# afalchetti/monorfs

Hardware: AMD Instinct MI355X
Metric: PHD updates/sec (particles x components x measurements) (higher is better)
Workload: dtype f64; 1 GPU; RB-PHD-SLAM SlamUpdate, BASELINE config B: 2048 particles/GPU x 512 components x 64 measurements, PRM3D pixel-range model, prior weights 'survey', state resident in HBM; particles_per_gpu=2048, components=512, measurements=64, max_quantity=600, parallelism=particles sharded x1

## Files before the change

### monorfs_amd/csrc/phd_alpha.h

```cpp
#pragma once
#include "phd_device.h"


__device__ __forceinline__ int pk_get(unsigned int perm, int i) { return (int) ((perm >> (4 * i)) & 15u); }

__device__ __forceinline__ unsigned int pk_set(unsigned int perm, int i, int v)
{
	return (perm & ~(15u << (4 * i))) | ((unsigned int) v << (4 * i));
}

__device__ __forceinline__ unsigned int pk_reverse(unsigned int perm, int from, int to)
{
	for (int i = from, j = to - 1; i < j; i++, j--) {
		int vi = pk_get(perm, i), vj = pk_get(perm, j);
		perm = pk_set(pk_set(perm, i, vj), j, vi);
	}
	return perm;
}

__device__ __forceinline__ bool pk_last(unsigned int perm, int n)
{
	for (int i = 1; i < n; i++) {
		if (pk_get(perm, i - 1) < pk_get(perm, i)) return false;
	}
// ... 360 lines not shown
	};
	auto store_node = [&](int slot, const int (&mx)[NT], unsigned int fr, int parent, int er, int ec) {
#pragma unroll
		for (int t = 0; t < NT; t++) {
			const int i = lane + 64 * t;
			if (i < n) nd.asg[(size_t) slot * nd.stride + i] = (unsigned char) mx[t];
			const unsigned long long w = ballot64((fr >> t) & 1u);
			if (lane == 0) nd.forced[slot * NT + t] = w;
		}
		int ne = 0;
		if (parent >= 0) {
			ne = nd.nelim[parent];
			for (int e = lane; e < ne; e += 64) nd.elist[slot * MURTY_ELCAP + e] = nd.elist[parent * MURTY_ELCAP + e];
		}
		if (lane == 0) {
			if (er >= 0 && ne < MURTY_ELCAP) nd.elist[slot * MURTY_ELCAP + ne] = (unsigned short) ((er << 8) | ec);
			nd.nelim[slot] = ne + ((er >= 0 && ne < MURTY_ELCAP) ? 1 : 0);
		}
		__threadfence_block();
	};

	{
		int slot = alloc();
		int mx[NT];
		bool solved = wave_hungarian<NT>(profit, n, lane, mx);
		if (!solved) {
#pragma unroll
			for (int t = 0; t < NT; t++) mx[t] = 0;
		}
		store_node(slot, mx, 0u, -1, -1, 0);
		double value = solved ? wave_assignment_value<NT>(profit, n, mx) : -INFINITY;
		frontier_add(value, solved ? slot : (slot | 0x10000));
	}

	while (fsize > 0) {
		const double value = ws.fkey[fsize - 1];
		const int    code  = ws.fnode[fsize - 1];
		fsize--;
		if (m >= MURTY_OUT || (ws.logcomp[m] - ws.logcomp[0] < -10)) break;
		if (lane == 0) ws.logcomp[m] = value;
		const int slot = code & 0xffff;
		hook(m, (code & 0x10000) != 0, [&](int row) { return (int) nd.asg[(size_t) slot * nd.stride + row]; });
		m++;
		lds_fence();
		if (code & 0x10000) continue;
		int pa[NT];
		unsigned int fr = 0, fc = 0;
		unsigned long long rem[NT];
		int R = 0;
#pragma unroll
		for (int t = 0; t < NT; t++) {
			const int i = lane + 64 * t;
			pa[t] = (i < n) ? nd.asg[(size_t) slot * nd.stride + i] : 0;
			const unsigned long long fw = nd.forced[slot * NT + t];
			if ((fw >> lane) & 1ull) fr |= 1u << t;
			const int left = n - 64 * t;
			const unsigned long long rows = (left >= 64) ? ~0ull : ((left <= 0) ? 0ull : ((1ull << left) - 1ull));
			rem[t] = ~fw & rows;
			R += __popcll(rem[t]);
		}
#pragma unroll
		for (int t = 0; t < NT; t++) {
			unsigned long long fw = ballot64((fr >> t) & 1u);
			while (fw) {
				const int l = __ffsll((long long) fw) - 1;
				fw &= fw - 1;
				const int col = __shfl(pa[t], l, 64);
				if (lane == (col & 63)) fc |= 1u << (col >> 6);
			}
		}
		const int pne = nd.nelim[slot];
		for (int c = 0; c < R - 1; c++) {
			int er = -1;
#pragma unroll
			for (int t = 0; t < NT; t++) {
				if (er < 0 && rem[t]) {
					er = 64 * t + __ffsll((long long) rem[t]) - 1;
					rem[t] &= rem[t] - 1;
				}
			}
			const int ec = spread_get<NT>(pa, er);
			for (int i = 0; i < n; i++) {
				const int  pai = spread_get<NT>(pa, i);
				const bool fi  = __shfl((int) fr, i & 63, 64) & (1 << (i >> 6));
#pragma unroll
				for (int t = 0; t < NT; t++) {
					const int k = lane + 64 * t;
					if (k < n) {
						double v = profit[i * n + k];
						if (fi) v = (k == pai) ? 1.0 : -INFINITY;
						else if ((fc >> t) & 1u) v = -INFINITY;
						nd.reduced[i * n + k] = v;
					}
				}
			}
			__threadfence_block();
			for (int e = lane; e < pne; e += 64) {
				const int ed = nd.elist[slot * MURTY_ELCAP + e];
				nd.reduced[(ed >> 8) * n + (ed & 255)] = -INFINITY;
			}
			if (lane == 0) nd.reduced[er * n + ec] = -INFINITY;
			__threadfence_block();
			int mx[NT];
			const bool solved = wave_hungarian<NT>(nd.reduced, n, lane, mx);
			if (solved) {
				const int cs = alloc();
				store_node(cs, mx, fr, slot, er, ec);
				frontier_add(wave_assignment_value<NT>(profit, n, mx), cs);
			}
			if (lane == (er & 63)) fr |= 1u << (er >> 6);
			if (lane == (ec & 63)) fc |= 1u << (ec >> 6);
		}
		if (lane == 0) ws.freelist[nfree] = slot;
		nfree++;
		lds_fence();
	}
	return m;
}

template <int TAG, class Hook>
__device__ __forceinline__ int wave_murty_any(const MurtyLds& ws, const MurtyWs& nd, int n, int lane, Hook hook)
{
	if (n <= 64) return wave_murty<1, TAG>(ws, nd, n, lane, hook);
	if (n <= 128) return wave_murty<2, TAG>(ws, nd, n, lane, hook);
	return wave_murty<4, TAG>(ws, nd, n, lane, hook);
}

__device__ void jacobian_p(const DevParams& prm, const PoseD& pose, const double m[3], double* Jp)
{
	if (prm.linear2d) {
		for (int i = 0; i < 18; i++) Jp[i] = 0.0;
		Jp[0] = -1.0; Jp[7] = -1.0;
		return;
	}
	const double diff[3] = {m[0] - pose.t[0], m[1] - pose.t[1], m[2] - pose.t[2]};
	double l[3];
	to_local(pose, diff, l);
	const double f = prm.focal;
	const double mag = ((l[2] > 0) ? 1.0 : -1.0) * sqrt(l[0] * l[0] + l[1] * l[1] + l[2] * l[2]);
	const double jp[9] = {f / l[2], 0, -f * l[0] / (l[2] * l[2]),  0, f / l[2], -f * l[1] / (l[2] * l[2]),
	                      l[0] / mag, l[1] / mag, l[2] / mag};
	double rc[9], jlocal[18];
	conj_matrix(pose, rc);
	const double cross[9] = {0, -diff[2], diff[1],  diff[2], 0, -diff[0],  -diff[1], diff[0], 0};
#pragma unroll
	for (int i = 0; i < 3; i++) {
#pragma unroll
		for (int j = 0; j < 3; j++) {
			double acc = 0;
#pragma unroll
			for (int k = 0; k < 3; k++) acc += (-1.0 * rc[i * 3 + k]) * cross[k * 3 + j];
			jlocal[i * 6 + j]     = -1.0 * rc[i * 3 + j];
			jlocal[i * 6 + 3 + j] = acc;
		}
	}
#pragma unroll
	for (int i = 0; i < 3; i++) {
#pragma unroll
		for (int j = 0; j < 6; j++) {
			double acc = 0;
#pragma unroll
			for (int k = 0; k < 3; k++) acc += jp[i * 3 + k] * jlocal[k * 6 + j];
			Jp[i * 6 + j] = acc;
		}
	}
}

__device__ __forceinline__ double pair_gradient(const DevParams& prm, const double* nu, const double* Jp, int t)
{
	double acc = 0;
#pragma unroll
	for (int b = 0; b < 3; b++) {
		double u = 0;
#pragma unroll
		for (int e = 0; e < 3; e++) u += nu[e] * prm.Rinv[e * 3 + b];
		acc += u * Jp[b * 6 + t];
	}
	return acc;
}

template <class Hook>
__device__ int cluster_enumerate_wave(const double* mat, int n, int modelsize, double* logcomp, int lane, Hook hook)
{
	int measurestart = n;
	for (int i = 0; i < n; i++) {
		if (i >= modelsize) { measurestart = i; break; }
	}
	unsigned int perm = pk_reverse(0x43210u, measurestart, n);
	int m = 0;
	for (;;) {
		double v = 0;
		for (int i = 0; i < n; i++) v += mat[i * 5 + pk_get(perm, i)];
		if (m < MURTY_OUT) {
			if (lane == 0) logcomp[m] = v;
			hook(m, perm);
			m++;
		}
		if (pk_last(perm, n)) break;
		perm = pk_next(perm, n, measurestart);
	}
	lds_fence();
	return m;
}

__global__ __launch_bounds__(64) void k_test_pairing(MurtyNodes* nodes, char* bigws, const double* matrix, int n, int mode, int modelsize,
                                                     int maxcount, int* assignments, double* values, int* count)
{
	__shared__ double lds[MURTY_LDS_DOUBLES + 2];
	const int lane = threadIdx.x;
	const MurtyLds ws = murty_lds(lds);
	const MurtyWs nd = (n <= MURTY_NMAX) ? murty_ws_particle(nodes) : murty_ws_carve(bigws, n);
	for (int i = lane; i < MURTY_OUT; i += 64) ws.logcomp[i] = 1e300;
	const int stride = (mode == 1) ? 5 : n;
	double* mat = (mode == 1) ? nd.reduced : nd.profit;
	for (int e = lane; e < n * n; e += 64) mat[(e / n) * stride + (e % n)] = matrix[e];
	lds_fence();
	int m;
	if (mode == 1) {
		m = cluster_enumerate_wave(mat, n, modelsize, ws.logcomp, lane, [&](int k, unsigned int perm) {
			if (k < maxcount && lane < n) assignments[k * n + lane] = pk_get(perm, lane);
		});
	}
	else {
		m = wave_murty_any<0>(ws, nd, n, lane, [&](int k, bool unsolved, auto colof) {
			if (k >= maxcount) return;
			for (int r = lane; r < n; r += 64) assignments[k * n + r] = unsolved ? -1 : colof(r);
		});
	}
	for (int k = lane; k < m && k < maxcount; k += 64) values[k] = ws.logcomp[k];
	if (lane == 0) *count = m;
}

#define ALPHA_JL 256

struct AlphaLds {
	int zs, red, lm, pick, scr;
	int p1_keyw, p1_sortw, p1_dw, p1_sortsrc, p1_selidx, ns;
	int p2_tile, p2_part;
	int p3_zh, p3_pdj, p3_lmd, p3_res, p3_adj, p3_adjT, p3_mem, p3_int, p3_x;
	int bytes;
};

__host__ __device__ inline AlphaLds alpha_lds(int MP, int ncap)
{
	const int JL = ALPHA_JL, MW = MP / 64;
	AlphaLds l;
	l.zs   = 0;
	l.red  = l.zs + 3 * MP;
	l.lm   = l.red + 256;
	l.pick = l.lm + 3 * JL;
	l.scr  = l.pick + JL / 2;
	int ns = 2;
	while (ns < ncap) ns <<= 1;
	l.ns = ns;
	l.p1_keyw = l.scr;
	l.p1_sortw = l.p1_keyw + ncap;
	l.p1_dw = l.p1_sortw + ns;
	l.p1_sortsrc = l.p1_dw + JL;
	l.p1_selidx = l.p1_sortsrc + (ns + JL + 1) / 2;
	int ph1 = l.p1_selidx + ns / 2 - l.scr;
	l.p2_tile = l.scr;
	l.p2_part = l.scr;
	int ph2 = 0;
	l.p3_zh = l.scr;
	l.p3_pdj = l.p3_zh + 3 * JL;
	l.p3_lmd = l.p3_pdj + JL;
	l.p3_res = l.p3_lmd + JL;
	l.p3_adj = l.p3_res + JL;
	l.p3_adjT = l.p3_adj + JL * MW;
	l.p3_mem = l.p3_adjT + MP * (JL / 64);
	l.p3_int = l.p3_mem + 2 * JL;
	l.p3_x   = l.p3_int + (3 * JL + MP + 1) / 2;
	int xs = 25 * 4 > MURTY_LDS_DOUBLES ? 25 * 4 : MURTY_LDS_DOUBLES;
	int ph3 = l.p3_x + xs + 2 - l.scr;
	int mx = ph1 > ph2 ? ph1 : ph2;
	mx = mx > ph3 ? mx : ph3;
	l.bytes = (l.scr + mx) * 8;
	return l;
}

#define QGRAD_WAVE_DOUBLES (25 + 5 * 18 + 120 * 6 + 120 + 9)
#define QGRAD_LDS_DOUBLES (4 * QGRAD_WAVE_DOUBLES)
#define QGRAD_G2_CLUSTERS 64
#define QGRAD_G2_WEIGHTS 384
#define QGRAD_HDR 10
#ifndef DENS_JL
#define DENS_JL 128
#endif
struct AlphaSlab {
	static constexpr int lm = 0, dw = 3, zh = 4, lpd = 7, res = 8, adj = 9, ints = 17, lmd = 19, memL = 20, memZ = 21, cnt = 22, total = 23;
	static constexpr int partc = 0, partp = 13;
	static constexpr int i_pick = 0, i_dsrc = 1, i_labl = 2, i_roots = 3;
	static constexpr int g_hdr = 0, g_jpall = g_hdr + QGRAD_HDR * ALPHA_JL, g_elist = g_jpall + 18 * ALPHA_JL;
};
static_assert(AlphaSlab::lm + 3 <= AlphaSlab::dw && AlphaSlab::dw + 1 <= AlphaSlab::zh && AlphaSlab::zh + 3 <= AlphaSlab::lpd &&
              AlphaSlab::lpd + 1 <= AlphaSlab::res && AlphaSlab::res + 1 <= AlphaSlab::adj && AlphaSlab::adj + 4 <= AlphaSlab::ints &&
              AlphaSlab::ints + (AlphaSlab::i_roots + 2) / 2 <= AlphaSlab::lmd && AlphaSlab::lmd + 1 <= AlphaSlab::memL &&
              AlphaSlab::memL + 1 <= AlphaSlab::memZ && AlphaSlab::memZ + 1 <= AlphaSlab::cnt && AlphaSlab::cnt + 1 <= AlphaSlab::total &&
              AlphaSlab::partc + 4 <= AlphaSlab::partp && AlphaSlab::partp + 4 <= AlphaSlab::total,
              "AlphaSlab: the Jcap-scaled arrays that are live together overlap, or pass the total");
__host__ __device__ inline size_t alpha_jscratch_doubles(int Jcap) { return (size_t) AlphaSlab::total * Jcap; }
__device__ __forceinline__ unsigned int my_xcd() { return __builtin_amdgcn_s_getreg((3 << 11) | 20) & 15u; }

template <int MW>
__device__ __forceinline__ bool has_detection(const unsigned long long* adj, int j)
{
	bool has = false;
#pragma unroll
	for (int b = 0; b < MW; b++) has |= adj[(size_t) j * MW + b] != 0;
	return has;
}

template <int ZB, bool QUASI, bool GRAD = false, int TAG = 0, bool DEPTH = false>
__device__ __forceinline__ void alpha_assoc_body(const DevParams& prm, const StepBufs& a, int ncap, double* smem, double* gws = nullptr,
                                                 int* helper_go = nullptr)
{
	constexpr int MP = ZB * 64;
	constexpr int MW = ZB;
	constexpr int JL = ALPHA_JL;
	const AlphaLds lay = alpha_lds(MP, ncap);
	double* zs   = smem + lay.zs;
	double* red  = smem + lay.red;
	double* etab = red;
	__shared__ int s_J, s_changed, s_nroots, s_big;
	__shared__ double s_ccount, s_total;
	__shared__ int s_ebump, s_g2lds;
	__shared__ double s_g2[GRAD ? QGRAD_G2_CLUSTERS * QGRAD_HDR + QGRAD_G2_WEIGHTS : 2];
	if (GRAD && threadIdx.x == 0) s_g2lds = 0;

	const int p = a.p0 + blockIdx.x, tid = threadIdx.x, lane = tid & 63, wv = tid >> 6;
	const int M = a.M, cap = a.cap;
	const MixView vout = bank_view(a, SEL_OUT);
	const Bank bin = bank_of(a, SEL_IN);
	const int no = QUASI ? 0 : vout.count[p];
	const size_t sbo = (size_t) p * cap;
	const PoseD pose = load_pose(QUASI ? a.qposes + (size_t) p * 7 : bin.poses + (size_t) p * 7);

	for (int k = tid; k < MP * 3; k += 256) zs[k] = (k < M * 3) ? a.z[k] : 0.0;
	unsigned int helper_word = 0;
	if (!QUASI && helper_go && tid == 0) helper_word = __hip_atomic_load(a.dsync + 3 * (size_t) p, __ATOMIC_RELAXED, __HIP_MEMORY_SCOPE_AGENT);

	PHD_STAMP_DECL;
	PHD_STAMP(0);
	double* keyw    = smem + lay.p1_keyw;
	double* sortw   = smem + lay.p1_sortw;
	int*    sortsrc = (int*) (smem + lay.p1_sortsrc);
	auto block_sum = [&](double v) {
		red[tid] = v;
		__syncthreads();
		for (int s = 128; s > 0; s >>= 1) {
			if (tid < s) red[tid] += red[tid + s];
			__syncthreads();
		}
		double r = red[0];
		__syncthreads();
		return r;
	};
	double wpart = 0;
	for (int c = tid; c < no; c += 256) {
		double wc = a.outw[sbo + c];
		keyw[c] = wc;
		wpart += wc;
	}
	{
		double e = block_sum(wpart);
		if (fabs(e - rint(e)) <= 1e-9 * fmax(1.0, fabs(e))) {
			if (tid == 0) {
				double q = 0;
				for (int c = 0; c < no; c++) q += keyw[c];
				s_ccount = q;
			}
			__syncthreads();
			e = s_ccount;
		}
		if (tid == 0) {
			s_ccount = e;
			int J = (int) e;
			if (J < 0) J = 0;
			if (J > a.Jcap) {
				atomicOr(a.flags, PHD_FLAG_J_OVERFLOW);
				J = a.Jcap;
			}
			s_J = QUASI ? min(a.qJ, a.Jcap) : J;
		}
	}
	PHD_STAMP(1);
	__syncthreads();
	const int J = s_J;
	if (J >= 1 && J <= no) {
		constexpr int HB = 500;
		int* const hist   = (int*) red;
		int* const selidx = (int*) (smem + lay.p1_selidx);
		int* const tl     = sortsrc;
		int& s_T = hist[HB];
		int& s_above = hist[HB + 1];
		int& s_nt = hist[HB + 2];
		int& s_ntaken = hist[HB + 3];
		const unsigned int hbase = (unsigned int) (((unsigned long long) __double_as_longlong(prm.minw) << 1) >> 49);
		auto bin_of = [&](double w) {
			const unsigned int k = (unsigned int) (((unsigned long long) __double_as_longlong(w) << 1) >> 49);
			return (int) min(max((int) k - (int) hbase, 0), HB - 1);
		};
		for (int t = tid; t < HB + 4; t += 256) hist[t] = 0;
		__syncthreads();
		for (int c = tid; c < no; c += 256) atomicAdd(&hist[bin_of(keyw[c])], 1);
		__syncthreads();
		if (wv == 0) {
			int cq[8], mine = 0;
#pragma unroll
			for (int q = 0; q < 8; q++) { const int b = 511 - (8 * lane + q); cq[q] = (b < HB) ? hist[b] : 0; mine += cq[q]; }
			int incl = mine;
#pragma unroll
			for (int o = 1; o < 64; o <<= 1) {
				const int y = __shfl_up(incl, o, 64);
				if (lane >= o) incl += y;
			}
			int run = incl - mine;
#pragma unroll
			for (int q = 0; q < 8; q++) {
				if (run < J && J <= run + cq[q]) { s_T = 511 - (8 * lane + q); s_above = run; }
				run += cq[q];
			}
		}
		__syncthreads();
		const int T = s_T, above = s_above, need = J - above;
		for (int c = tid; c < no; c += 256) {
			const int b = bin_of(keyw[c]);
			if (b > T) selidx[atomicAdd(&s_ntaken, 1)] = c;
			else if (b == T) tl[atomicAdd(&s_nt, 1)] = c;
		}
		__syncthreads();
		const int nt = s_nt;
		for (int t = tid; t < nt; t += 256) {
			const int ct = tl[t];
			const double wt = keyw[ct];
			int rank = 0;
			for (int u = 0; u < nt; u++) {
				const int cu = tl[u];
				const double wu = keyw[cu];
				rank += (wu > wt || (wu == wt && cu < ct)) ? 1 : 0;
			}
			if (rank < need) selidx[above + rank] = ct;
		}
		__syncthreads();
		for (int t = tid; t < J; t += 256) {
			const int ct = selidx[t];
			const double wt = keyw[ct];
			int rank = 0;
#pragma unroll 4
			for (int u = 0; u < J; u++) {
				const int cu = selidx[u];
				const double wu = keyw[cu];
				rank += (wu > wt || (wu == wt && cu < ct)) ? 1 : 0;
			}
			sortw[rank]   = wt;
			sortsrc[rank] = ct;
		}
		__syncthreads();
	}
	else if (!QUASI && J > no) {
		unsigned long long* sv = (unsigned long long*) sortw;
		int NS = 2;
		while (NS < no) NS <<= 1;
		for (int t = tid; t < NS; t += 256) sv[t] = (t < no) ? prune_pack(keyw[t], t) : 0ull;
		__syncthreads();
		prune_bitonic(sv, NS, tid);
		for (int r = tid; r + 1 < no; r += 256) {
			const unsigned long long kb = prune_kbits(sv[r]);
			if (prune_kbits(sv[r + 1]) != kb || (r > 0 && prune_kbits(sv[r - 1]) == kb)) continue;
			int e = r + 2;
			while (e < no && prune_kbits(sv[e]) == kb) e++;
			for (int x = r + 1; x < e; x++) {
				unsigned long long vx = sv[x];
				int sx = prune_slot(vx);
				double wx = keyw[sx];
				int y = x - 1;
				while (y >= r) {
					int sy = prune_slot(sv[y]);
					if (keyw[sy] > wx || (keyw[sy] == wx && sy < sx)) break;
					sv[y + 1] = sv[y];
					y--;
				}
				sv[y + 1] = vx;
			}
		}
		__syncthreads();
		for (int r = tid; r < no; r += 256) sortsrc[r] = prune_slot(sv[r]);
		__syncthreads();
		for (int r = tid; r < no; r += 256) sortw[r] = keyw[sortsrc[r]];
		__syncthreads();
	}
	PHD_STAMP(2);
	const bool inlds = J <= JL;
	const int  JS = inlds ? JL : a.Jcap;
	double* gj = a.jscratch + (size_t) p * alpha_jscratch_doubles(a.Jcap);
	double* lm   = inlds ? smem + lay.lm     : gj + AlphaSlab::lm * (size_t) JS;
	double* dw   = inlds ? smem + lay.p1_dw  : gj + AlphaSlab::dw * (size_t) JS;
	double* zh   = inlds ? smem + lay.p3_zh  : gj + AlphaSlab::zh * (size_t) JS;
	double* lpd  = inlds ? smem + lay.p3_pdj : gj + AlphaSlab::lpd * (size_t) JS;
	double* lmd  = inlds ? smem + lay.p3_lmd : gj + AlphaSlab::lmd * (size_t) JS;
	double* res  = inlds ? smem + lay.p3_res : gj + AlphaSlab::res * (size_t) JS;
	unsigned long long* adj = (unsigned long long*) (inlds ? smem + lay.p3_adj : gj + AlphaSlab::adj * (size_t) JS);
	int* gi      = (int*) (gj + AlphaSlab::ints * (size_t) JS);
	int* pick    = inlds ? (int*) (smem + lay.pick) : gi + AlphaSlab::i_pick * JS;
	int* dsrc    = inlds ? sortsrc + lay.ns : gi + AlphaSlab::i_dsrc * JS;
	int* labl    = inlds ? (int*) (smem + lay.p3_int) : gi + AlphaSlab::i_labl * JS;
	int* roots   = inlds ? labl + JL : gi + AlphaSlab::i_roots * JS;
	int* cnt     = inlds ? labl + 2 * JL : (int*) (gj + AlphaSlab::cnt * (size_t) JS);
	unsigned long long* memL = (unsigned long long*) (inlds ? smem + lay.p3_mem : gj + AlphaSlab::memL * (size_t) JS);
	unsigned long long* memZ = (unsigned long long*) (inlds ? smem + lay.p3_mem + JL : gj + AlphaSlab::memZ * (size_t) JS);
	int* labz    = (int*) (smem + lay.p3_int) + 3 * JL;
	double* xreg = smem + lay.p3_x;
	const bool straight = J <= no && (J == 0 || !(sortw[0] - 1 > sortw[J - 1]));
	if (QUASI) {}
	else if (straight) {
		for (int j = tid; j < J; j += 256) pick[j] = sortsrc[j];
	}
	else if (tid == 0) {
		int ia = 0, id = 0, nd = 0;
		for (int j = 0; j < J; j++) {
			bool takeorig;
			if (ia < no && id < nd) takeorig = !(dw[id] > sortw[ia]);
			else takeorig = ia < no;
			double wpick;
			int    src;
			if (takeorig) { wpick = sortw[ia]; src = sortsrc[ia]; ia++; }
			else          { wpick = dw[id];    src = dsrc[id];    id++; }
			dw[nd]   = wpick - 1;
			dsrc[nd] = src;
			nd++;
			pick[j] = src;
		}
	}
	__threadfence_block();
	__syncthreads();
	for (int j = tid; j < J; j += 256) {
		if (QUASI) {
			lm[j] = a.qlm[j * 3]; lm[JS + j] = a.qlm[j * 3 + 1]; lm[2 * JS + j] = a.qlm[j * 3 + 2];
		}
		else {
			int c = pick[j];
			const double2* rc = (const double2*) (vout.rec + (sbo + c) * MIX_REC);
			const double2 r0 = rc[0], r1 = rc[1];
			double l0 = r0.y, l1 = r1.x, l2 = r1.y;
			lm[j] = l0; lm[JS + j] = l1; lm[2 * JS + j] = l2;
			double* glm = a.alm + (size_t) p * 3 * a.Jcap;
			glm[j] = l0; glm[a.Jcap + j] = l1; glm[2 * a.Jcap + j] = l2;
		}
	}
	if (!QUASI && helper_go) {
		if (tid == 0) { a.aJ[p] = J; a.account[p] = s_ccount; }
		asm volatile("s_waitcnt vmcnt(0)" ::: "memory");
	}
	__threadfence_block();
	__syncthreads();
	if (!QUASI && helper_go && tid == 0) {
		const int go = (J > 0 && J <= DENS_JL && helper_word == ((a.dstamp << 4) | my_xcd())) ? 1 : 0;
		__hip_atomic_store(a.dsync + 3 * (size_t) p + 1, 2u * a.dstamp + (unsigned int) go, __ATOMIC_RELAXED, __HIP_MEMORY_SCOPE_AGENT);
		*helper_go = go;
#ifdef PHD_STAMPS
		if (a.stamps && a.stamp_kernel == 5) { a.stamps[(size_t) p * 16 + 12] = go; a.stamps[(size_t) p * 16 + 13] = (double) wall_clock64(); }
#endif
	}

	PHD_STAMP(3);
	{
		double* mats = xreg;

		constexpr int JW = JL / 64;
		unsigned long long* adjT = (unsigned long long*) (smem + lay.p3_adjT);
		for (int j = tid; j < J; j += 256) {
			double m[3] = {lm[j], lm[JS + j], lm[2 * JS + j]}, z[3], l[3];
			measure_perfect(prm, pose, m, z, l);
			const float dz = (!QUASI && DEPTH) ? depth_at(prm, z) : 0.0f;
			zh[j] = z[0]; zh[JS + j] = z[1]; zh[2 * JS + j] = z[2];
			const double pdv = QUASI ? prm.pd : detection_probability_m<!QUASI && DEPTH>(prm, z, dz);
			lpd[j] = log(pdv);
			lmd[j] = log(1 - pdv);
#pragma unroll
			for (int b = 0; b < MW; b++) adj[(size_t) j * MW + b] = 0;
			labl[j] = j;
			cnt[j]  = 0;
			memL[j] = 0;
			memZ[j] = 0;
		}
		for (int k = tid; k < M; k += 256) labz[k] = J + k;
		for (int t = tid; t < MP * JW; t += 256) adjT[t] = 0;
		if (tid == 0) { s_nroots = 0; s_big = 0; }
		__threadfence_block();
		__syncthreads();
		{
			double kx[ZB], ky[ZB], kz[ZB];
#pragma unroll
			for (int b = 0; b < ZB; b++) {
				const int k = b * 64 + lane;
				kx[b] = zs[k * 3]; ky[b] = zs[k * 3 + 1]; kz[b] = zs[k * 3 + 2];
			}
			const double g2 = QUASI ? prm.g2_quasi : prm.g2_assoc;
			for (int j = wv; j < J; j += 4) {
				const double h0 = zh[j], h1 = zh[JS + j], h2 = zh[2 * JS + j];
#pragma unroll
				for (int b = 0; b < ZB; b++) {
					const int k = b * 64 + lane;
					const bool gated = k < M && quad_gen(prm.Rinv, h0 - kx[b], h1 - ky[b], h2 - kz[b]) < g2;
					const unsigned long long bal = ballot64(gated);
					if (lane == 0) adj[(size_t) j * MW + b] = bal;
					if (gated && inlds) atomicOr(&adjT[(size_t) k * JW + (j >> 6)], 1ull << (j & 63));
				}
			}
		}
		__threadfence_block();
		__syncthreads();

		PHD_STAMP(4);
		for (int it = 0; it < J + M + 1; it++) {
			if (tid == 0) s_changed = 0;
			__syncthreads();
			for (int j = tid; j < J; j += 256) {
				int l = labl[j];
#pragma unroll
				for (int b = 0; b < MW; b++) {
					unsigned long long bits = adj[(size_t) j * MW + b];
					while (bits) {
						int k = b * 64 + __ffsll((long long) bits) - 1;
						bits &= bits - 1;
						l = min(l, labz[k]);
					}
				}
				if (l < labl[j]) { labl[j] = l; s_changed = 1; }
			}
			__threadfence_block();
			__syncthreads();
			for (int k = tid; k < M; k += 256) {
				int l = labz[k];
				if (inlds) {
#pragma unroll
					for (int b = 0; b < JW; b++) {
						unsigned long long bits = adjT[(size_t) k * JW + b];
						while (bits) {
							int j = b * 64 + __ffsll((long long) bits) - 1;
							bits &= bits - 1;
							l = min(l, labl[j]);
						}
					}
				}
				else {
					for (int j = 0; j < J; j++) {
						if ((adj[(size_t) j * MW + (k >> 6)] >> (k & 63)) & 1ull) l = min(l, labl[j]);
					}
				}
				if (l < labz[k]) { labz[k] = l; s_changed = 1; }
			}
			__threadfence_block();
			__syncthreads();
			if (!s_changed) break;
			__syncthreads();
		}
		for (int j = tid; j < J; j += 256) {
			const int r = labl[j];
			const int slot = atomicAdd(&cnt[r], 1) & 0xffff;
			if (slot < 5) atomicOr(&memL[r], (unsigned long long) j << (12 * slot));
		}
		for (int k = tid; k < M; k += 256) {
			const int r = labz[k];
			if (r < J) {
				const int slot = atomicAdd(&cnt[r], 0x10000) >> 16;
				if (slot < 5) atomicOr(&memZ[r], (unsigned long long) k << (12 * slot));
			}
		}
		if (wv == 0) {
			int nr = 0;
			for (int j0 = 0; j0 < J; j0 += 64) {
				const int j = j0 + lane;
				bool isroot = false;
				if (j < J) {
					const bool has = has_detection<MW>(adj, j);
					isroot = has && labl[j] == j;
				}
				unsigned long long bal = ballot64(isroot);
				if (isroot) roots[nr + __popcll(bal & lanemask_lt())] = j;
				nr += __popcll(bal);
			}
			if (lane == 0) s_nroots = nr;
		}
		exp_tab_init(etab, tid);
		__syncthreads();
		const int nroots = s_nroots;
		const double logmult = prm.logRmult;

		PHD_STAMP(5);
		if (GRAD) {
			if (tid == 0) s_big = 1;
		}
		else if (J >= 5) {
			for (int ri = tid; ri < nroots; ri += 256) {
				const int root = roots[ri];
				const int cn = cnt[root];
				const int nl = cn & 0xffff, nz = cn >> 16;
				if (nl + nz > 5) {
					res[ri] = NAN;
					s_big = 1;
					continue;
				}
				const unsigned long long Lp = pk_sort5(memL[root], nl), Zp = pk_sort5(memZ[root], nz);
				double E[25];
#pragma unroll
				for (int e = 0; e < 25; e++) E[e] = (e % 6 == 0) ? 1.0 : 0.0;
				double rsum = 0;
				bool dead = false;
#pragma unroll
				for (int x = 0; x < 4; x++) {
					if (x < nl) {
						const int j = (int) ((Lp >> (12 * x)) & 4095);
						const double md = lmd[j], lp = lpd[j];
						const double h0 = zh[j], h1 = zh[JS + j], h2 = zh[2 * JS + j];
						double D[4], rx = md;
#pragma unroll
						for (int y = 0; y < 4 - x; y++) {
							D[y] = -INFINITY;
							if (y < nz) {
								const int k = (int) ((Zp >> (12 * y)) & 4095);
								if ((adj[(size_t) j * MW + (k >> 6)] >> (k & 63)) & 1ull) {
									double dist = sqrt(quad_gen(prm.Rinv, h0 - zs[k * 3], h1 - zs[k * 3 + 1], h2 - zs[k * 3 + 2]));
									D[y] = lp + logmult - 0.5 * dist * dist;
									rx = fmax(rx, D[y]);
								}
							}
						}
						if (rx == -INFINITY) dead = true;
						else {
							rsum += rx;
							E[x * 6] = exp_neg(md - rx, etab);
#pragma unroll
							for (int y = 0; y < 4 - x; y++) {
								if (y < nz) E[x * 5 + 4 - y] = (D[y] == -INFINITY) ? 0.0 : exp_neg(D[y] - rx, etab);
							}
						}
					}
				}
#pragma unroll
				for (int y = 0; y < 4; y++) {
					if (y < nz) {
						E[(4 - y) * 6] = prm.kappa;
#pragma unroll
						for (int x = 0; x < 4 - y; x++) {
							if (x < nl) E[(4 - y) * 5 + x] = 1.0;
						}
					}
				}
				double f[32];
#pragma unroll
				for (int m = 0; m < 32; m++) f[m] = 0;
				f[0] = 1;
#pragma unroll
				for (int i = 0; i < 5; i++) {
#pragma unroll
					for (int m = 0; m < 32; m++) {
						if (__builtin_popcount(m) == i) {
#pragma unroll
							for (int c = 0; c < 5; c++) {
								if (!((m >> c) & 1)) f[m | (1 << c)] = fma(f[m], E[i * 5 + c], f[m | (1 << c)]);
							}
						}
					}
				}
				res[ri] = dead ? -INFINITY : rsum + log(f[31]);
			}
		}
		else if (wv == 0) {
			for (int r0 = 0; r0 < nroots; r0 += 64) {
				int ri = r0 + lane;
				if (ri < nroots) {
					int root = roots[ri];
					unsigned long long Lp = 0, Zp = 0;
					int nl = 0, nz = 0, nrow = 0;
					for (int j = root; j < J; j++) {
						if (labl[j] == root) { if (nl < 5) Lp |= (unsigned long long) j << (12 * nl); nl++; }
					}
					for (int k = 0; k < M; k++) {
						if (labz[k] == root) { if (nz < 5) Zp |= (unsigned long long) k << (12 * nz); nz++; }
					}
					nrow = nl + nz;
					if (nrow > 5) {
						res[ri] = NAN;
						s_big = 1;
					}
					else {
						double* mat = mats + lane;
						for (int e = 0; e < 25; e++) mat[e * 4] = -INFINITY;
						for (int x = 0; x < nl; x++) {
							int j = (int) ((Lp >> (12 * x)) & 4095);
							for (int y = 0; y < nz; y++) {
								int k = (int) ((Zp >> (12 * y)) & 4095);
								if ((adj[(size_t) j * MW + (k >> 6)] >> (k & 63)) & 1ull) {
									double dist = sqrt(quad_gen(prm.Rinv, zh[j] - zs[k * 3], zh[JS + j] - zs[k * 3 + 1],
									                            zh[2 * JS + j] - zs[k * 3 + 2]));
									mat[(x * 5 + y) * 4] = lpd[j] + logmult - 0.5 * dist * dist;
								}
							}
							mat[(x * 5 + nz + x) * 4] = lmd[j];
						}
						for (int y = 0; y < nz; y++) {
							mat[((nl + y) * 5 + y) * 4] = prm.logkappa;
							for (int x = 0; x < nl; x++) mat[((nl + y) * 5 + nz + x) * 4] = 0;
						}
						res[ri] = cluster_enumerate(mat, 4, nrow, J);
					}
				}
			}
		}
		__syncthreads();
		if (GRAD && gws && inlds) {
			double* const wsm = gws + wv * QGRAD_WAVE_DOUBLES;
			double* const gmat = wsm;
			double* const gjp = wsm + 25;
			double (*gdv)[6] = (double (*)[6]) (wsm + 25 + 5 * 18);
			double* const glc = wsm + 25 + 5 * 18 + 120 * 6;
			int* const gL = (int*) (glc + 120);
			int* const gZ = gL + 8;
			double* const jpall = gj + AlphaSlab::g_jpall;
			double* const elist = gj + AlphaSlab::g_elist;
			const int ecap = (int) alpha_jscratch_doubles(a.Jcap) - AlphaSlab::g_elist;
			const int gt = (lane < 6) ? lane : 0;
			if (tid == 0) s_ebump = 0;
			if (ecap > 0) {
				for (int j = tid; j < J; j += 256) {
					const double m3[3] = {lm[j], lm[JS + j], lm[2 * JS + j]};
					jacobian_p(prm, pose, m3, jpall + (size_t) j * 18);
				}
			}
			__threadfence_block();
			__syncthreads();
			const bool pairfast = J >= 5 && ecap > 0;
			if (pairfast) {
				for (int ri = tid; ri < nroots; ri += 256) {
					const int root = roots[ri];
					if (cnt[root] != 0x10001) continue;
					const int j = (int) (memL[root] & 4095), k = (int) (memZ[root] & 4095);
					double* const h = gj + (size_t) ri * QGRAD_HDR;
					const bool gated = (adj[(size_t) j * MW + (k >> 6)] >> (k & 63)) & 1ull;
					double c0 = -INFINITY;
					if (gated) {
						double dist = sqrt(quad_gen(prm.Rinv, zh[j] - zs[k * 3], zh[JS + j] - zs[k * 3 + 1], zh[2 * JS + j] - zs[k * 3 + 2]));
						c0 = lpd[j] + logmult - 0.5 * dist * dist;
					}
					c0 = (0.0 + c0) + 0.0;
					const double c1 = (0.0 + lmd[j]) + prm.logkappa;
					const double mx = fmax(fmax(-INFINITY, c0), c1);
					const bool finite = !(isinf(mx) && mx < 0);
					double lse = -INFINITY, w0 = c0, w1 = c1;
					if (finite) {
						double value = 0;
						value += exp(c0 - mx);
						value += exp(c1 - mx);
						lse = mx + log(value);
						w0 = exp_neg(c0 - mx, etab);
						w1 = exp_neg(c1 - mx, etab);
					}
					res[ri] = lse;
					const int off = atomicAdd(&s_ebump, 2);
					if (off + 2 > ecap) { h[0] = -2; continue; }
					elist[off] = w0;
					elist[off + 1] = w1;
					double G[6] = {0, 0, 0, 0, 0, 0};
					if (finite && gated) {
						const double nu[3] = {zs[k * 3] - zh[j], zs[k * 3 + 1] - zh[JS + j], zs[k * 3 + 2] - zh[2 * JS + j]};
						const double* Jp = jpall + (size_t) j * 18;
#pragma unroll
						for (int t = 0; t < 6; t++) G[t] = w0 * (0.0 + pair_gradient(prm, nu, Jp, t));
					}
					h[0] = 2.0;
#pragma unroll
					for (int t = 0; t < 6; t++) h[1 + t] = G[t];
					h[7] = (double) off;
					h[8] = finite ? 1.0 : 0.0;
				}
			}
			PHD_STAMP(9);
			for (int ri = wv; ri < nroots; ri += 4) {
				const int root = roots[ri];
				if (pairfast && cnt[root] == 0x10001) continue;
				double* const h = gj + (size_t) ri * QGRAD_HDR;
				int nl = 0, nz = 0;
				for (int j0 = root; j0 < J; j0 += 64) {
					const int j = j0 + lane;
					const bool in = j < J && labl[j] == root;
					const unsigned long long bal = ballot64(in);
					const int pos = nl + __popcll(bal & lanemask_lt());
					if (in && pos < 6) gL[pos] = j;
					nl += __popcll(bal);
				}
				for (int k0 = 0; k0 < M; k0 += 64) {
					const int k = k0 + lane;
					const bool in = k < M && labz[k] == root;
					const unsigned long long bal = ballot64(in);
					const int pos = nz + __popcll(bal & lanemask_lt());
					if (in && pos < 6) gZ[pos] = k;
					nz += __popcll(bal);
				}
				const int nrow = nl + nz;
				if (nrow > 5) {
					if (lane == 0) h[0] = -1;
					continue;
				}
				lds_fence();
				if (lane < nrow * nrow) {
					const int x = lane / nrow, y = lane - x * nrow;
					double v = -INFINITY;
					if (x < nl) {
						const int j = gL[x];
						if (y < nz) {
							const int k = gZ[y];
							if ((adj[(size_t) j * MW + (k >> 6)] >> (k & 63)) & 1ull) {
								double dist = sqrt(quad_gen(prm.Rinv, zh[j] - zs[k * 3], zh[JS + j] - zs[k * 3 + 1], zh[2 * JS + j] - zs[k * 3 + 2]));
								v = lpd[j] + logmult - 0.5 * dist * dist;
							}
						}
						else if (y - nz == x) v = lmd[j];
					}
					else {
						if (y < nz) { if (y == x - nl) v = prm.logkappa; }
						else v = 0;
					}
					gmat[x * 5 + y] = v;
				}
				if (ecap <= 0) {
					if (lane == 0) h[0] = -2;
					continue;
				}
				int mcount;
				double mx = -INFINITY, value = 0;
				if (nrow <= J) {
					double* const pgt = gjp;
					const int npair = nl * nz;
					bool g = false;
					{
						const int pr = lane / 6, t = lane - 6 * pr;
						if (pr < npair) {
							const int x = pr / nz, y = pr - x * nz;
							const int j = gL[x], k = gZ[y];
							g = (adj[(size_t) j * MW + (k >> 6)] >> (k & 63)) & 1ull;
							double v = 0;
							if (g) {
								const double nu[3] = {zs[k * 3] - zh[j], zs[k * 3 + 1] - zh[JS + j], zs[k * 3 + 2] - zh[2 * JS + j]};
								v = pair_gradient(prm, nu, jpall + (size_t) j * 18, t);
							}
							pgt[(x * 4 + y) * 6 + t] = v;
						}
					}
					const unsigned long long gb = ballot64(g);
					unsigned int gmask = 0;
					for (int pr = 0; pr < npair; pr++) {
						if ((gb >> (6 * pr)) & 1ull) gmask |= 1u << ((pr / nz) * 4 + (pr % nz));
					}
					lds_fence();
					mcount = 1;
					for (int i = 2; i <= nrow; i++) mcount *= i;
					double vv[2] = {-INFINITY, -INFINITY};
#pragma unroll
// ... 539 lines not shown
	double* const etab = partcl + (JL / 64) * 256;
	int* const s_wc = (int*) (etab + EXPTAB_N);
	double* red = tile;

	const int p = (pin >= 0) ? pin : a.p0 + blockIdx.x, tid = threadIdx.x, lane = tid & 63, wv = tid >> 6;
	const int cap = a.cap;
	const MixView vin = bank_view(a, SEL_IN), vout = bank_view(a, SEL_OUT);
	const Bank bin = bank_of(a, SEL_IN);
	const Bank bout = bank_of(a, SEL_OUT);
	const int n = vin.count[p], nb = a.born_count[p], no = vout.count[p];
	const int np = n + nb;
	const size_t sbi = in_base(a, p), sbo = (size_t) p * cap;
	const int J = a.aJ[p];
	const int JS = a.Jcap;
	const double* lm = a.alm + (size_t) p * 3 * JS;
	double* gj = a.jscratch + (size_t) p * alpha_jscratch_doubles(a.Jcap);
	double* partp = (J <= JL) ? partpl : gj + AlphaSlab::partp * (size_t) JS;
	double* partc = (J <= JL) ? partcl : gj + AlphaSlab::partc * (size_t) JS;
	const double* wcopy = a.wcopy + (size_t) p * (cap + a.Mcap);
	const int* cover = a.cover + sbo;
	if (!pre) exp_tab_init(etab, tid);
	__syncthreads();

	double plog_part = 0, clog_part = 0, pcount_part = pre ? pre_pcount : 0.0;
	{
		const int JB = (J + 63) >> 6;
		const bool pair = PHD_DENS_PAIR && J > 0 && J <= JL;
		constexpr int ULIST = (JL / 64) * 256 * 8 / 2;
		unsigned short* const ulist = (unsigned short*) partcl;
		int* const ucnt = (int*) partpl;
		if (!pair) {
			for (int i = tid; i < JB * 256; i += 256) { partp[i] = 0; partc[i] = 0; }
		}
		int  plj[2] = {1, 1}, pcc[2] = {0, 0}, pstep[2] = {256, 256};
		unsigned int pj[2][2] = {};
		bool ptwo[2] = {false, false};
		double pacc[2][2] = {}, pcacc[2][2] = {};
		if (pair && !triple) {
#pragma unroll
			for (int b = 0; b < 2; b++) {
				const int rem = min(64, J - b * 64);
				if (rem <= 0) continue;
				const int S = (rem > 32) ? 64 : ((rem <= 1) ? 1 : (1 << (32 - __clz(rem - 1))));
				ptwo[b] = S > 1;
				const int lj = ptwo[b] ? (S >> 1) : 1, G = 64 / lj, jl = lane & (lj - 1);
				plj[b] = lj;
				pcc[b] = wv * G + lane / lj;
				pstep[b] = 4 * G;
				pj[b][0] = 8u * (b * 64 + ((jl < rem) ? jl : 0));
				pj[b][1] = 8u * (b * 64 + ((lj + jl < rem) ? lj + jl : 0));
			}
		}
		auto pair_block = [&](const int b, const bool first, const int cend) {
			double xa[3], xb[3];
			unsigned int oa = pj[b][0], ob = pj[b][1];
			asm volatile("" : "+v"(oa), "+v"(ob));
#pragma unroll
			for (int t = 0; t < 3; t++) {
				const char* const row = (const char*) (lm + t * JS);
				xa[t] = *(const double*) (row + oa);
				xb[t] = *(const double*) (row + ob);
			}
			auto visit = [&](const int cc, const bool two) {
				const double* tt = tile + cc * DENS_REC;
				double g[DENS_REC - 1];
#pragma unroll
				for (int t = 0; t < DENS_REC - 1; t++) g[t] = (t < 10 || first) ? tt[t] : 0;
				const double e1 = exp_pair(gauss_logw(g, xa[0] - g[0], xa[1] - g[1], xa[2] - g[2]), etab);
				const double e2 = two ? exp_pair(gauss_logw(g, xb[0] - g[0], xb[1] - g[1], xb[2] - g[2]), etab) : 0.0;
				if (first) {
					pacc[b][0] += e1;
					pcacc[b][0] = fma(g[10], e1, pcacc[b][0]);
					if (two) {
						pacc[b][1] += e2;
						pcacc[b][1] = fma(g[10], e2, pcacc[b][1]);
					}
				}
				else {
					pcacc[b][0] += e1;
					if (two) pcacc[b][1] += e2;
				}
			};
			if (ptwo[b]) {
				for (int cc = pcc[b]; cc < cend; cc += pstep[b]) visit(cc, true);
			}
			else {
				for (int cc = pcc[b]; cc < cend; cc += pstep[b]) visit(cc, false);
			}
		};
		auto triple_tile = [&](const bool first, const int cend) {
			double xa[3], xb[3], xc[3];
			const int jl = lane & 31;
			unsigned int oa = 8u * jl, ob = 8u * (32 + jl), oc = 8u * ((64 + jl < J) ? 64 + jl : 64);
			asm volatile("" : "+v"(oa), "+v"(ob), "+v"(oc));
#pragma unroll
			for (int t = 0; t < 3; t++) {
				const char* const row = (const char*) (lm + t * JS);
				xa[t] = *(const double*) (row + oa);
				xb[t] = *(const double*) (row + ob);
				xc[t] = *(const double*) (row + oc);
			}
			for (int cc = wv * 2 + (lane >> 5); cc < cend; cc += 8) {
				const double* tt = tile + cc * DENS_REC;
				double g[DENS_REC - 1];
#pragma unroll
				for (int t = 0; t < DENS_REC - 1; t++) g[t] = (t < 10 || first) ? tt[t] : 0;
				const double e1 = exp_pair(gauss_logw(g, xa[0] - g[0], xa[1] - g[1], xa[2] - g[2]), etab);
				const double e2 = exp_pair(gauss_logw(g, xb[0] - g[0], xb[1] - g[1], xb[2] - g[2]), etab);
				const double e3 = exp_pair(gauss_logw(g, xc[0] - g[0], xc[1] - g[1], xc[2] - g[2]), etab);
				if (first) {
					pacc[0][0] += e1;
					pacc[0][1] += e2;
					pacc[1][0] += e3;
					pcacc[0][0] = fma(g[10], e1, pcacc[0][0]);
					pcacc[0][1] = fma(g[10], e2, pcacc[0][1]);
					pcacc[1][0] = fma(g[10], e3, pcacc[1][0]);
				}
				else {
					pcacc[0][0] += e1;
					pcacc[0][1] += e2;
					pcacc[1][0] += e3;
				}
			}
		};
		for (int src = 0; src < 2; src++) {
			int total = (src == 0) ? np : no;
			const bool listed = src == 1 && triple && no <= ULIST;
			if (listed) {
				const int nwin = (no + 255) >> 8;
				unsigned int mine = 0;
				unsigned int co = 4u * (unsigned int) tid;
				asm volatile("" : "+v"(co));
				for (int i = 0; i < nwin; i++) {
					const int c = i * 256 + tid;
					const bool other = c < no && !*(const int*) ((const char*) cover + co + 1024u * i);
					const unsigned long long bal = ballot64(other);
					if (lane == 0) ucnt[i * 4 + wv] = __popcll(bal);
					mine |= (other ? 1u : 0u) << i;
				}
				__syncthreads();
				int base = 0;
				for (int i = 0; i < nwin; i++) {
					const bool other = (mine >> i) & 1u;
					const unsigned long long bal = ballot64(other);
					int slot = base + __popcll(bal & lanemask_lt());
					for (int q = 0; q < wv; q++) slot += ucnt[i * 4 + q];
					if (other) ulist[slot] = (unsigned short) (i * 256 + tid);
					base += ucnt[i * 4] + ucnt[i * 4 + 1] + ucnt[i * 4 + 2] + ucnt[i * 4 + 3];
				}
				total = base;
				__syncthreads();
			}
			for (int c0 = 0; c0 < total; c0 += DENS_TILE) {
				int c = (DENS_TILE < 256 && tid >= DENS_TILE) ? total : c0 + tid;
				int cend;
				if (src == 0) {
					if (pre && c0 == 0 && c < n) {
						const double w = tile[tid * DENS_REC + 11];
						tile[tid * DENS_REC + 10] = (w > 0) ? wcopy[c] / w : 0.0;
					}
					else if (c < total) {
						double w, m[3], P[6], Pi[6], det;
						if (c < n) {
							load_comp(vin.rec + (sbi + c) * MIX_REC, w, m, P);
							pcount_part += w;
						}
						else {
							const double* bm = a.born_mean + ((size_t) p * a.Mcap + (c - n)) * 3;
							w = prm.birthw;
							m[0] = bm[0]; m[1] = bm[1]; m[2] = bm[2];
#pragma unroll
							for (int t = 0; t < 6; t++) P[t] = prm.birthP[t];
						}
						inv_sym3(P, Pi, det);
						gauss_record(w, m, Pi, PHD_INV_2PI / sqrt(fabs(det)), tile + tid * DENS_REC);
						tile[tid * DENS_REC + 10] = (w > 0) ? wcopy[c] / w : 0.0;
					}
					cend = min(DENS_TILE, total - c0);
				}
				else if (listed) {
					cend = min(DENS_TILE, total - c0);
					if (tid < cend) {
						double w, m[3], P[6], Pi[6], det;
						load_comp(vout.rec + (sbo + ulist[c0 + tid]) * MIX_REC, w, m, P);
						inv_sym3(P, Pi, det);
						gauss_record(w, m, Pi, PHD_INV_2PI / sqrt(fabs(det)), tile + tid * DENS_REC);
					}
				}
				else {
					const bool other = c < total && !cover[c];
					const unsigned long long bal = ballot64(other);
					if (lane == 0) s_wc[wv] = __popcll(bal);
					__syncthreads();
					int slot = __popcll(bal & lanemask_lt());
					for (int q = 0; q < wv; q++) slot += s_wc[q];
					cend = s_wc[0] + s_wc[1] + s_wc[2] + s_wc[3];
					if (other) {
						double w, m[3], P[6], Pi[6], det;
						load_comp(vout.rec + (sbo + c) * MIX_REC, w, m, P);
						inv_sym3(P, Pi, det);
						gauss_record(w, m, Pi, PHD_INV_2PI / sqrt(fabs(det)), tile + slot * DENS_REC);
					}
				}
				__syncthreads();
				if constexpr (triple) {
					if (src == 0) triple_tile(true, cend);
					else          triple_tile(false, cend);
				}
				else if (pair) {
					if (src == 0) {
						pair_block(0, true, cend);
						if (JB > 1) pair_block(1, true, cend);
					}
					else {
						pair_block(0, false, cend);
						if (JB > 1) pair_block(1, false, cend);
					}
				}
				for (int jb = 0; jb < JB && cend > 0 && !pair && !triple; jb++) {
					const int rem = min(64, J - jb * 64);
					const int LJ  = (rem > 32) ? 64 : ((rem <= 1) ? 1 : (1 << (32 - __clz(rem - 1))));
					const int G   = 64 / LJ, g = lane / LJ, jl = lane & (LJ - 1);
					const bool jv = jl < rem;
					const int  j  = jb * 64 + jl;
					const double x0 = jv ? lm[j] : 0, x1 = jv ? lm[JS + j] : 0, x2 = jv ? lm[2 * JS + j] : 0;
					auto dens = [&](int cc) {
						const double* tt = tile + cc * DENS_REC;
						return exp_pair(gauss_logw(tt, x0 - tt[0], x1 - tt[1], x2 - tt[2]), etab);
					};
					double acc = 0, acc2 = 0, cacc = 0, cacc2 = 0;
					int cc = wv * G + g;
					const int step = 4 * G;
					if (src == 0) {
						for (; cc + step < cend; cc += 2 * step) {
							const double e1 = dens(cc), e2 = dens(cc + step);
							acc  += e1;
							acc2 += e2;
							cacc  = fma(tile[cc * DENS_REC + 10], e1, cacc);
							cacc2 = fma(tile[(cc + step) * DENS_REC + 10], e2, cacc2);
						}
						if (cc < cend) {
							const double e1 = dens(cc);
							acc += e1;
							cacc = fma(tile[cc * DENS_REC + 10], e1, cacc);
						}
						partp[(jb * 4 + wv) * 64 + lane] += acc + acc2;
						partc[(jb * 4 + wv) * 64 + lane] += cacc + cacc2;
					}
					else {
						for (; cc + step < cend; cc += 2 * step) {
							acc  += dens(cc);
							acc2 += dens(cc + step);
						}
						if (cc < cend) acc += dens(cc);
						partc[(jb * 4 + wv) * 64 + lane] += acc + acc2;
					}
				}
				__syncthreads();
			}
			if constexpr (triple) {
				double* const part = (src == 0) ? partp : partc;
				const double v0 = (src == 0) ? pacc[0][0] : pcacc[0][0], v1 = (src == 0) ? pacc[0][1] : pcacc[0][1];
				const double v2 = (src == 0) ? pacc[1][0] : pcacc[1][0];
				const bool upper = (lane & 32) != 0;
				double keep = upper ? v1 : v0;
				keep += __shfl_xor(upper ? v0 : v1, 32, 64);
				part[wv * 64 + lane] = keep;
				const double both = v2 + __shfl_xor(v2, 32, 64);
				part[(4 + wv) * 64 + lane] = upper ? 0.0 : both;
			}
			else if (pair) {
				double* const part = (src == 0) ? partp : partc;
#pragma unroll
				for (int b = 0; b < 2; b++) {
					if (b >= JB) continue;
					const double v0 = (src == 0) ? pacc[b][0] : pcacc[b][0], v1 = (src == 0) ? pacc[b][1] : pcacc[b][1];
					double keep = v0;
					if (ptwo[b]) {
						const bool odd = (lane & plj[b]) != 0;
						keep = odd ? v1 : v0;
						keep += __shfl_xor(odd ? v0 : v1, plj[b], 64);
					}
					part[(b * 4 + wv) * 64 + lane] = keep;
				}
			}
			__threadfence_block();
			__syncthreads();
			const double* part = (src == 0) ? partp : partc;
			for (int jb = wv; jb < JB; jb += 4) {
				const int rem = min(64, J - jb * 64);
				const int LJ  = (rem > 32) ? 64 : ((rem <= 1) ? 1 : (1 << (32 - __clz(rem - 1))));
				const int jl = lane & (LJ - 1);
				double v = part[(jb * 4 + 0) * 64 + lane] + part[(jb * 4 + 1) * 64 + lane] + part[(jb * 4 + 2) * 64 + lane] +
				           part[(jb * 4 + 3) * 64 + lane];
				for (int o = LJ; o < 64; o <<= 1) v += __shfl_xor(v, o, 64);
				if (lane < LJ && jl < rem) {
					if (src == 0) plog_part += log(v);
					else          clog_part += log(v);
				}
			}
			__syncthreads();
		}
	}
	auto block_sum = [&](double v) {
		red[tid] = v;
		__syncthreads();
		for (int s = 128; s > 0; s >>= 1) {
			if (tid < s) red[tid] += red[tid + s];
			__syncthreads();
		}
		double r = red[0];
		__syncthreads();
		return r;
	};
	const double plog = block_sum(plog_part);
	const double clog = block_sum(clog_part);
	const double pcount = block_sum(pcount_part) + nb * prm.birthw;
	if (tid == 0) {
		const double ccount = a.account[p];
		double ratio = (plog - pcount) - (clog - ccount);
		if (meet) {
			__hip_atomic_store(a.ratio + p, ratio, __ATOMIC_RELAXED, __HIP_MEMORY_SCOPE_AGENT);
			s_wc[0] = alpha_meet(a, p, true, ratio) ? 1 : 0;
		}
		else {
			double alpha = exp(a.setll[p] + ratio);
			a.alpha[p] = alpha;
			bout.weights[p] = bin.weights[p] * alpha;
		}
	}
	if (!meet) return true;
	__syncthreads();
	return s_wc[0] != 0;
}

__device__ __forceinline__ bool alpha_density_body(const DevParams& prm, const StepBufs& a, double* pool, int pin = -1, bool meet = false,
                                                   bool pre = false, double pre_pcount = 0.0)
{
	const int J = a.aJ[(pin >= 0) ? pin : a.p0 + blockIdx.x];
	if (PHD_DENS_PAIR >= 2 && J > 80 && J <= 96) return alpha_density_body_t<true>(prm, a, pool, pin, meet, pre, pre_pcount);
	return alpha_density_body_t<false>(prm, a, pool, pin, meet, pre, pre_pcount);
}

__global__ __launch_bounds__(256, PHD_DENS_WAVES) void k_alpha_density(const DevParams prm, const StepBufs a)
{
	__shared__ __align__(16) double pool[DENS_LDS_DOUBLES];
	PHD_TL_BEGIN;
	PHD_SET_PRIO(PHD_DENSE_PRIO);
	alpha_density_body(prm, a, pool);
	PHD_TL_END(4);
}
```

Measured before the change: 123.1 billion PHD updates/s.

## Cut block barriers in alpha association: wave-shuffle sums, bucketed top-J select, double-buffered flag

Replaces the eight-barrier shared-memory tree reduction with a single-wave shuffle reduction. It rewrites the top-J component selection so candidates are scattered into histogram-bucket order via prefix offsets, with ranks computed only within each bucket instead of across all J. It moves the scratch initialisation and record loads ahead of the gating loop, and splits the measure/log work across two threads per landmark when J is at most 128. The label-propagation loop double-buffers its changed flag to remove a barrier per iteration. Together these aim to reduce barriers and quadratic ranking cost, but they reorder floating-point summation and rely on pre and bucket bounds being correct.

```diff
diff --git a/monorfs_amd/csrc/phd_alpha.h b/monorfs_amd/csrc/phd_alpha.h
--- a/monorfs_amd/csrc/phd_alpha.h
+++ b/monorfs_amd/csrc/phd_alpha.h
@@ -686,6 +686,23 @@
 __host__ __device__ inline size_t alpha_jscratch_doubles(int Jcap) { return (size_t) AlphaSlab::total * Jcap; }
 __device__ __forceinline__ unsigned int my_xcd() { return __builtin_amdgcn_s_getreg((3 << 11) | 20) & 15u; }
 
+__device__ __forceinline__ double block_tree_sum(double* red, double v, int tid)
+{
+	const int lane = tid & 63;
+	red[tid] = v;
+	__syncthreads();
+	if (tid < 64) {
+		double x = (red[lane] + red[lane + 128]) + (red[lane + 64] + red[lane + 192]);
+#pragma unroll
+		for (int s = 32; s > 0; s >>= 1) x += __shfl_down(x, s, 64);
+		if (lane == 0) red[0] = x;
+	}
+	__syncthreads();
+	const double r = red[0];
+	__syncthreads();
+	return r;
+}
+
 template <int MW>
 __device__ __forceinline__ bool has_detection(const unsigned long long* adj, int j)
 {
@@ -706,7 +723,7 @@
 	double* zs   = smem + lay.zs;
 	double* red  = smem + lay.red;
 	double* etab = red;
-	__shared__ int s_J, s_changed, s_nroots, s_big;
+	__shared__ int s_J, s_changed[2], s_nroots, s_big;
 	__shared__ double s_ccount, s_total;
 	__shared__ int s_ebump, s_g2lds;
 	__shared__ double s_g2[GRAD ? QGRAD_G2_CLUSTERS * QGRAD_HDR + QGRAD_G2_WEIGHTS : 2];
@@ -729,17 +746,7 @@
 	double* keyw    = smem + lay.p1_keyw;
 	double* sortw   = smem + lay.p1_sortw;
 	int*    sortsrc = (int*) (smem + lay.p1_sortsrc);
-	auto block_sum = [&](double v) {
-		red[tid] = v;
-		__syncthreads();
-		for (int s = 128; s > 0; s >>= 1) {
-			if (tid < s) red[tid] += red[tid + s];
-			__syncthreads();
-		}
-		double r = red[0];
-		__syncthreads();
-		return r;
-	};
+	auto block_sum = [&](double v) { return block_tree_sum(red, v, tid); };
 	double wpart = 0;
 	for (int c = tid; c < no; c += 256) {
 		double wc = a.outw[sbo + c];
@@ -775,11 +782,10 @@
 		constexpr int HB = 500;
 		int* const hist   = (int*) red;
 		int* const selidx = (int*) (smem + lay.p1_selidx);
-		int* const tl     = sortsrc;
+		int* const pre    = (int*) (smem + lay.p1_dw);
 		int& s_T = hist[HB];
 		int& s_above = hist[HB + 1];
 		int& s_nt = hist[HB + 2];
-		int& s_ntaken = hist[HB + 3];
 		const unsigned int hbase = (unsigned int) (((unsigned long long) __double_as_longlong(prm.minw) << 1) >> 49);
 		auto bin_of = [&](double w) {
 			const unsigned int k = (unsigned int) (((unsigned long long) __double_as_longlong(w) << 1) >> 49);
@@ -802,43 +808,33 @@
 			int run = incl - mine;
 #pragma unroll
 			for (int q = 0; q < 8; q++) {
-				if (run < J && J <= run + cq[q]) { s_T = 511 - (8 * lane + q); s_above = run; }
+				const int b = 511 - (8 * lane + q);
+				if (b < HB) pre[b] = run;
+				if (run < J && J <= run + cq[q]) { s_T = b; s_above = run; s_nt = cq[q]; }
 				run += cq[q];
 			}
 		}
 		__syncthreads();
-		const int T = s_T, above = s_above, need = J - above;
+		const int T = s_T, above = s_above;
+		const int ncand = above + s_nt;
 		for (int c = tid; c < no; c += 256) {
 			const int b = bin_of(keyw[c]);
-			if (b > T) selidx[atomicAdd(&s_ntaken, 1)] = c;
-			else if (b == T) tl[atomicAdd(&s_nt, 1)] = c;
+			if (b >= T) selidx[pre[b] + atomicSub(&hist[b], 1) - 1] = c;
 		}
 		__syncthreads();
-		const int nt = s_nt;
-		for (int t = tid; t < nt; t += 256) {
-			const int ct = tl[t];
-			const double wt = keyw[ct];
-			int rank = 0;
-			for (int u = 0; u < nt; u++) {
-				const int cu = tl[u];
-				const double wu = keyw[cu];
-				rank += (wu > wt || (wu == wt && cu < ct)) ? 1 : 0;
-			}
-			if (rank < need) selidx[above + rank] = ct;
-		}
-		__syncthreads();
-		for (int t = tid; t < J; t += 256) {
-			const int ct = selidx[t];
-			const double wt = keyw[ct];
-			int rank = 0;
+		for (int e = tid; e < ncand; e += 256) {
+			const int ce = selidx[e];
+			const double we = keyw[ce];
+			const int b = bin_of(we);
+			const int lo = pre[b], hi = (b == T) ? ncand : pre[b - 1];
+			int rank = lo;
 #pragma unroll 4
-			for (int u = 0; u < J; u++) {
+			for (int u = lo; u < hi; u++) {
 				const int cu = selidx[u];
 				const double wu = keyw[cu];
-				rank += (wu > wt || (wu == wt && cu < ct)) ? 1 : 0;
-			}
-			sortw[rank]   = wt;
-			sortsrc[rank] = ct;
+				rank += (wu > we || (wu == we && cu < ce)) ? 1 : 0;
+			}
+			if (rank < J) { sortw[rank] = we; sortsrc[rank] = ce; }
 		}
 		__syncthreads();
 	}
@@ -918,14 +914,27 @@
 	}
 	__threadfence_block();
 	__syncthreads();
+	constexpr int JW = JL / 64;
+	unsigned long long* adjT = (unsigned long long*) (smem + lay.p3_adjT);
+	for (int k = tid; k < M; k += 256) labz[k] = J + k;
+	for (int t = tid; t < MP * JW; t += 256) adjT[t] = 0;
+	if (tid == 0) { s_nroots = 0; s_big = 0; s_changed[0] = 0; }
 	for (int j = tid; j < J; j += 256) {
+		double2 r0 = {0.0, 0.0}, r1 = {0.0, 0.0};
+		if (!QUASI) {
+			const double2* rc = (const double2*) (vout.rec + (sbo + pick[j]) * MIX_REC);
+			r0 = rc[0]; r1 = rc[1];
+		}
+#pragma unroll
+		for (int b = 0; b < MW; b++) adj[(size_t) j * MW + b] = 0;
+		labl[j] = j;
+		cnt[j]  = 0;
+		memL[j] = 0;
+		memZ[j] = 0;
 		if (QUASI) {
 			lm[j] = a.qlm[j * 3]; lm[JS + j] = a.qlm[j * 3 + 1]; lm[2 * JS + j] = a.qlm[j * 3 + 2];
 		}
 		else {
-			int c = pick[j];
-			const double2* rc = (const double2*) (vout.rec + (sbo + c) * MIX_REC);
-			const double2 r0 = rc[0], r1 = rc[1];
 			double l0 = r0.y, l1 = r1.x, l2 = r1.y;
 			lm[j] = l0; lm[JS + j] = l1; lm[2 * JS + j] = l2;
 			double* glm = a.alm + (size_t) p * 3 * a.Jcap;
@@ -951,26 +960,20 @@
 	{
 		double* mats = xreg;
 
-		constexpr int JW = JL / 64;
-		unsigned long long* adjT = (unsigned long long*) (smem + lay.p3_adjT);
-		for (int j = tid; j < J; j += 256) {
+		const bool pair = J <= 128;
+		for (int t = tid; t < (pair ? 256 : J); t += 256) {
+			const int j = pair ? (t & 127) : t;
+			if (j >= J) continue;
 			double m[3] = {lm[j], lm[JS + j], lm[2 * JS + j]}, z[3], l[3];
 			measure_perfect(prm, pose, m, z, l);
 			const float dz = (!QUASI && DEPTH) ? depth_at(prm, z) : 0.0f;
-			zh[j] = z[0]; zh[JS + j] = z[1]; zh[2 * JS + j] = z[2];
 			const double pdv = QUASI ? prm.pd : detection_probability_m<!QUASI && DEPTH>(prm, z, dz);
-			lpd[j] = log(pdv);
-			lmd[j] = log(1 - pdv);
-#pragma unroll
-			for (int b = 0; b < MW; b++) adj[(size_t) j * MW + b] = 0;
-			labl[j] = j;
-			cnt[j]  = 0;
-			memL[j] = 0;
-			memZ[j] = 0;
-		}
-		for (int k = tid; k < M; k += 256) labz[k] = J + k;
-		for (int t = tid; t < MP * JW; t += 256) adjT[t] = 0;
-		if (tid == 0) { s_nroots = 0; s_big = 0; }
+			if (!pair || t < 128) {
+				zh[j] = z[0]; zh[JS + j] = z[1]; zh[2 * JS + j] = z[2];
+				lpd[j] = log(pdv);
+			}
+			if (!pair || t >= 128) lmd[j] = log(1 - pdv);
+		}
 		__threadfence_block();
 		__syncthreads();
 		{
@@ -998,8 +1001,7 @@
 
 		PHD_STAMP(4);
 		for (int it = 0; it < J + M + 1; it++) {
-			if (tid == 0) s_changed = 0;
-			__syncthreads();
+			int* const changed = &s_changed[it & 1];
 			for (int j = tid; j < J; j += 256) {
 				int l = labl[j];
 #pragma unroll
@@ -1011,10 +1013,11 @@
 						l = min(l, labz[k]);
 					}
 				}
-				if (l < labl[j]) { labl[j] = l; s_changed = 1; }
+				if (l < labl[j]) { labl[j] = l; *changed = 1; }
 			}
 			__threadfence_block();
 			__syncthreads();
+			if (tid == 0) s_changed[(it & 1) ^ 1] = 0;
 			for (int k = tid; k < M; k += 256) {
 				int l = labz[k];
 				if (inlds) {
@@ -1033,12 +1036,11 @@
 						if ((adj[(size_t) j * MW + (k >> 6)] >> (k & 63)) & 1ull) l = min(l, labl[j]);
 					}
 				}
-				if (l < labz[k]) { labz[k] = l; s_changed = 1; }
+				if (l < labz[k]) { labz[k] = l; *changed = 1; }
 			}
 			__threadfence_block();
 			__syncthreads();
-			if (!s_changed) break;
-			__syncthreads();
+			if (!*changed) break;
 		}
 		for (int j = tid; j < J; j += 256) {
 			const int r = labl[j];
@@ -2184,17 +2186,7 @@
 			__syncthreads();
 		}
 	}
-	auto block_sum = [&](double v) {
-		red[tid] = v;
-		__syncthreads();
-		for (int s = 128; s > 0; s >>= 1) {
-			if (tid < s) red[tid] += red[tid + s];
-			__syncthreads();
-		}
-		double r = red[0];
-		__syncthreads();
-		return r;
-	};
+	auto block_sum = [&](double v) { return block_tree_sum(red, v, tid); };
 	const double plog = block_sum(plog_part);
 	const double clog = block_sum(clog_part);
 	const double pcount = block_sum(pcount_part) + nb * prm.birthw;
```

New measurement: 125.2 billion PHD updates/s (median of 6 runs). 1.7% higher.
